# parlance/ctcdecode

Hardware: AMD Instinct MI355X
Metric: utterances/sec at B=256 T=1000 V=29 beam=100 (higher is better)
Workload: dtype f32

## Files before the change

ctcdecode_amd/csrc/beam_core.h:

```cpp
#pragma once
#include <stddef.h>
#include <stdint.h>

#include "exact_math.h"
#include "exact_math_f64.h"
#include "lm_tables.h"
#include "stl_emul.h"
#if defined(CTC_ASSUME_CHECKED)
#include <cstdio>
#include <cstdlib>
#endif

#define CTC_RARE(x) __builtin_expect(!!(x), 0)
#if !defined(CTC_SPEC_UP)
#define CTC_SPEC_UP 1.5f
#endif
#if !defined(CTC_SPEC_DN)
#define CTC_SPEC_DN 0.7f
#endif
#if !defined(CTC_SPEC_OVER_SHIFT)
#define CTC_SPEC_OVER_SHIFT 2
#endif
#define CTC_USUAL(x) __builtin_expect(!!(x), 1)

namespace ctcbeam {

struct alignas(16) Int4v { int x, y, z, w; };

struct PoolNode {
  int32_t parent;
  float lpc;
  uint32_t cht;
  CTC_HD int ch() const { const uint32_t c = cht & 0xFFFFu; return c == 0xFFFFu ? -1 : (int)c; }
  CTC_HD static uint32_t pack(int ch, int tstep) { return ((uint32_t)ch & 0xFFFFu) | ((uint32_t)tstep << 16); }
};

struct EkWide { uint64_t k; uint32_t slot, pad; };
template <bool HUGE> struct EkOps;
template <> struct EkOps<false> {
  using E = uint64_t; using Pos = uint16_t;
  CTC_HD static E make(uint64_t key48v, int slot) { return (key48v << 16) | (uint64_t)slot; }
  CTC_HD static uint64_t key(const E &e) { return e >> 16; }
  CTC_HD static int slot(const E &e) { return (int)(e & 0xFFFFu); }
};
template <> struct EkOps<true> {
  using E = EkWide; using Pos = uint32_t;
  CTC_HD static E make(uint64_t key48v, int slot) { E e; e.k = key48v; e.slot = (uint32_t)slot; e.pad = 0; return e; }
  CTC_HD static uint64_t key(const E &e) { return e.k; }
  CTC_HD static int slot(const E &e) { return (int)e.slot; }
};

enum : uint32_t { T_SELF = 0, T_CHILD = 1, T_REVIVED = 2, T_HOLE = 3 };
enum : int { ST_OK = 0, ST_POOL_OVERFLOW = 1, ST_BAD_CONFIG = 2 };

constexpr int kMaxBeam = 16383;
constexpr int kMaxVocab = 65534;
constexpr int kIntMax = 0x7fffffff;

CTC_HD uint32_t ord_f32(float f) {
  const uint32_t u = ctcmath::f32_to_bits(f + 0.0f);
  return u ^ ((uint32_t)((int32_t)u >> 31) | 0x80000000u);
}
CTC_HD uint32_t ord_f32_raw(float f) {
  const uint32_t u = ctcmath::f32_to_bits(f);
  return u ^ ((uint32_t)((int32_t)u >> 31) | 0x80000000u);
}
CTC_HD float unord_f32(uint32_t k) {
  return ctcmath::bits_to_f32((k & 0x80000000u) ? (k ^ 0x80000000u) : ~k);
}
CTC_HD uint32_t mk_info(int ch, uint32_t type, int entry) {
  return ((uint32_t)(0xFFFF - (ch + 1)) << 16) | (type << 14) | (uint32_t)entry;
}
CTC_HD uint32_t info_type(uint32_t info) { return (info >> 14) & 3u; }
CTC_HD int info_entry(uint32_t info) { return (int)(info & 0x3FFFu); }
CTC_HD int info_ch(uint32_t info) { return 0xFFFF - (int)(info >> 16) - 1; }
CTC_HD uint64_t key48(uint32_t skey, uint32_t info) { return ((uint64_t)skey << 16) | (info >> 16); }
constexpr uint32_t kHoleInfo = T_HOLE << 14;

struct Beam {
  int *node, *par, *ch, *dep, *lcp, *via, *viaanc, *viach;
  int *up;
  float *bprev, *nbprev, *score, *lpc;
  int *lmst, *lmcl;
  int *acc_lo, *acc_hi;
  int *dn, *dmlo, *dmhi, *dfc;
  int *spc_lo, *spc_hi;
  int *spst, *spcl;
};
constexpr int kBeamArrays = 13, kBeamArraysLm = 12;

struct Dims {
  int K;
  int V;
  int Vc_max;
  int use_rank_table;
  int lm;
  CTC_HD int S_max() const { return K * (2 + Vc_max); }
};

enum {
  VAR_STATUS = 0, VAR_CUT, VAR_TAUC,
  VAR_INTO,
  VAR_FB0 = 4, VAR_FB1, VAR_FB2, VAR_FB3,
  VAR_TAU = 8, VAR_G, VAR_E,
  VAR_DANGER,
  VAR_PAR0 = 12,
  P_NPIN = 0, P_LCOUNT, P_NMAXKEY, P_NMINKEY, P_NCAND, P_SIZE = 8,
  VAR_SPEC = VAR_PAR0 + 2 * P_SIZE, SP_THR = 0, SP_WLOG, SP_ANCHOR, SP_PRED, SP_BEST, SP_MARGIN, SP_GAP, SP_ROWMAX,
  VAR_ROWMAX = VAR_SPEC + SP_ROWMAX,
  VAR_QSTAT = VAR_SPEC + 9,
  VAR_LMMISS = VAR_SPEC + 8,
  VAR_LMQ = VAR_SPEC + 10,
  VAR_HOTN = VAR_SPEC + 4,
  VAR_COUNT = VAR_SPEC + 12
};
constexpr int kBins = 1024;
constexpr int kBinsLog = 10;
constexpr int kListCap = 128;
constexpr int kSmallK = 128, kSmallV = 32;
constexpr int kMidK = 112, kMidVc = 40, kMidV = 10240;
constexpr int kHotCap = 256;
#if !defined(CTC_SERIAL_CUT)
#define CTC_SERIAL_CUT 12
#endif
constexpr int kSerialCut = CTC_SERIAL_CUT;
constexpr int kExpress = 32;
enum Event { EV_FRAMES, EV_CANDIDATES, EV_EXACT, EV_INTERNAL, EV_PINNED, EV_LPC_UPDATE, EV_DEAD_PARENT, EV_REVIVE_CAND, EV_REVIVED, EV_WALK,
             EV_WALK_HOPS, EV_FAST_SELECT, EV_SINGLE_KEY, EV_BUCKET_KEYS, EV_SPEC_OK, EV_SPEC_UNDER, EV_SPEC_OVER, EV_SPEC_OTHER, EV_SPEC_HOT,
             EV_SLOW_BELOW, EV_SLOW_CROWDED, EV_SLOW_SINGLE, EV_SLOW_ROUNDS, EV_TIE_FRAMES, EV_TIE_KEYS, EV_TIE_BIG, EV_WIDE_LIST, EV_HOT_LIST, EV_COUNT };

struct Work {
  Beam cur, nxt, beam0;
  size_t beam_blk;
  size_t beam_blk_far;
  size_t blk_via, blk_lm;
  int *e, *anc, *ostart, *cstart, *pinr, *revr;
  int *ancbuf, *acntbuf;
  uint32_t *hit;
  float *b_new, *nb_new, *sc_new, *rev_lpc;
  int *cch;
  float *clp;
  float *clpbuf;
  int16_t *rank_of;
  uint32_t *skey, *sinfo, *pos;
  int *surv;
  uint64_t *ek;
  uint16_t *lr;
  uint32_t *wpre;
  int *bins;
  int *hotge;
  int *lcpst;
  uint32_t *list;
  int *lslot;
  uint32_t *bitmap;
  int *fin, *sstack;
  int stage_skey;
  int *apos;
  int *vars;
};

template <class P>
CTC_HD P *carve_ptr(char *&p, size_t count) {
  P *r = reinterpret_cast<P *>(p);
  p += ((count * sizeof(P) + 15) / 16) * 16;
  return r;
}

template <int BIG, bool FARREP = false>
CTC_HD size_t carve(Work &w, char *base, char *far, const Dims &d, size_t *far_bytes) {
  char *p = base;
  char *q = far;
  constexpr bool deep = BIG >= 2;
  constexpr bool huge = BIG >= 3;
  const size_t K = (size_t)d.K, S = (size_t)d.S_max();
  const size_t Kr = ((K * 4 + 15) / 16) * 16;
  Beam *bs[2] = {&w.cur, &w.nxt};
  constexpr bool lm_far = BIG != 0;
  const size_t n_lm = d.lm ? (size_t)kBeamArraysLm : 0;
  w.beam_blk = (size_t)(kBeamArrays - (deep ? 3 : 0) + (lm_far ? 0 : n_lm)) * Kr;
  w.beam_blk_far = ((deep ? 3 : 0) + (lm_far ? n_lm : 0)) * Kr;
  w.blk_via = deep ? w.beam_blk_far : w.beam_blk;
  w.blk_lm = lm_far ? w.beam_blk_far : w.beam_blk;
  for (int i = 0; i < 2; ++i) {
    Beam &b = *bs[i];
    char *f = q + (size_t)i * w.beam_blk_far;
    b.node = carve_ptr<int>(p, K); b.par = carve_ptr<int>(p, K); b.ch = carve_ptr<int>(p, K);
    b.dep = carve_ptr<int>(p, K); b.lcp = carve_ptr<int>(p, K);
    char *&pv3 = deep ? f : p;
    b.via = carve_ptr<int>(pv3, K); b.viaanc = carve_ptr<int>(pv3, K); b.viach = carve_ptr<int>(pv3, K);
    b.up = carve_ptr<int>(p, K);
    b.bprev = carve_ptr<float>(p, K); b.nbprev = carve_ptr<float>(p, K); b.score = carve_ptr<float>(p, K);
    b.lpc = carve_ptr<float>(p, K);
    const size_t Kl = d.lm ? K : 0;
    char *&pl = lm_far ? f : p;
    b.lmst = carve_ptr<int>(pl, Kl); b.lmcl = carve_ptr<int>(pl, Kl); b.acc_lo = carve_ptr<int>(pl, Kl); b.acc_hi = carve_ptr<int>(pl, Kl);
    b.dn = carve_ptr<int>(pl, Kl); b.dmlo = carve_ptr<int>(pl, Kl); b.dmhi = carve_ptr<int>(pl, Kl); b.dfc = carve_ptr<int>(pl, Kl);
    b.spc_lo = carve_ptr<int>(pl, Kl); b.spc_hi = carve_ptr<int>(pl, Kl); b.spst = carve_ptr<int>(pl, Kl); b.spcl = carve_ptr<int>(pl, Kl);
  }
  q += 2 * w.beam_blk_far;
  w.beam0 = w.cur;
  w.e = carve_ptr<int>(p, K); w.ancbuf = carve_ptr<int>(p, 2 * K); w.acntbuf = carve_ptr<int>(p, 2 * K); w.anc = w.ancbuf;
  w.ostart = carve_ptr<int>(p, K);
  w.cstart = carve_ptr<int>(p, K);
  w.pinr = carve_ptr<int>(deep ? q : p, K);
  w.revr = carve_ptr<int>(deep ? q : p, K); w.hit = carve_ptr<uint32_t>(p, 2 * K);
  w.b_new = carve_ptr<float>(p, K); w.nb_new = carve_ptr<float>(p, K); w.sc_new = carve_ptr<float>(p, K);
  w.rev_lpc = carve_ptr<float>(deep ? q : p, K);
  w.cch = carve_ptr<int>(p, (size_t)d.Vc_max);
  w.clpbuf = carve_ptr<float>(p, 2 * (size_t)d.Vc_max); w.clp = w.clpbuf;
  w.rank_of = carve_ptr<int16_t>(p, d.use_rank_table ? (size_t)d.V : 0);
  w.skey = carve_ptr<uint32_t>(deep ? q : p, S);
  w.surv = carve_ptr<int>(p, 3 * K + 4);
  const size_t lcap = (d.K <= kSmallK && d.Vc_max <= kMidVc) ? (size_t)kHotCap + 64 : (size_t)kListCap + 4;
  w.bins = carve_ptr<int>(p, kBins + kBins / 16 + 4); w.list = carve_ptr<uint32_t>(p, lcap);
  w.lslot = carve_ptr<int>(p, lcap);
  w.hotge = carve_ptr<int>(p, lcap > (size_t)kListCap + 4 ? (size_t)kHotCap : 0);
#if defined(CTC_EXP_LCP_TABLE)
  w.lcpst = carve_ptr<int>(p, (lcap > (size_t)kListCap + 4 && !d.lm) ? (size_t)7 * kSmallK : 0);
#else
  w.lcpst = nullptr;
#endif
  w.bitmap = carve_ptr<uint32_t>(huge ? q : p, 2 * ((S + 63) / 64 + 17));
  w.wpre = huge ? carve_ptr<uint32_t>(q, (S + 63) / 64 + 2) : reinterpret_cast<uint32_t *>(w.bins);
  w.fin = carve_ptr<int>(BIG ? q : p, d.lm ? 2 * K : K);
  w.apos = carve_ptr<int>(BIG ? q : p, K);
  w.sstack = carve_ptr<int>(p, 3 * (2 * 32 + 2));
  w.vars = carve_ptr<int>(p, VAR_COUNT);
  w.sinfo = carve_ptr<uint32_t>(p, BIG ? K : S);
  w.pos = carve_ptr<uint32_t>(BIG ? q : p, K + 2);
  char *&rr = (BIG || FARREP) ? q : p;
  w.ek = carve_ptr<uint64_t>(rr, huge ? 2 * S : S); w.lr = carve_ptr<uint16_t>(rr, (2 * S + 2) * (huge ? 2 : 1));
  w.stage_skey = deep ? 0 : 1;
  if (far_bytes) *far_bytes = (size_t)(q - far);
  return (size_t)(p - base);
}

struct StreamState {
  int *hdr;
  int *arrays;
  int finish;
};
enum { SH_FRAMES = 0, SH_N, SH_POOL, SH_WLOG, SH_MAXKEY, SH_DANGER, SH_MINKEY,
       SH_SP_PRED, SH_SP_GAP, SH_SP_MARGIN,
       SH_WORDS = 12 };
constexpr int kStateArrays = 14;
constexpr int kStateArraysLm = kStateArrays + kBeamArraysLm;
CTC_HD int state_arrays(int lm) { return lm ? kStateArraysLm : kStateArrays; }

struct StepIn {
  int t;
  int Vc;
  int blank_rank;
  int identity;
  float blank_prob;
};


CTC_HD int div_p2(int v, int d) { return v >> __builtin_ctz((unsigned)d); }
CTC_HD int ceil_div_p2(int v, int d) { return div_p2(v + d - 1, d); }

CTC_HD double ctc_log_f64(double v) {
  return ctcmath::log_f64(v, ctcmath::tables64());
}

CTC_HD int ceil_log2_u32(uint32_t v) {
  return v <= 1u ? 0 : 32 - __builtin_clz(v - 1u);
}
CTC_HD int ceil_log2_u64(uint64_t v) {
  return v <= 1 ? 0 : 64 - __builtin_clzll(v - 1);
}

struct OutRefs {
  int32_t *tok, *ts;
  float *score;
  int32_t *len;
  int32_t *n_results;
  int K, T_stride;
  int32_t *c_hdr, *c_ent;
  uint32_t *c_rag;
  unsigned *c_count;
  unsigned c_cap;
  int32_t *m_hdr, *m_ent, *m_done;
  uint32_t *m_rag;
  unsigned m_cap;
};
enum : int { ST_COMPACT_OVERFLOW = 3, ST_INPUT_TIMEOUT = 4,
             ST_NEED_HOST = 5,
             ST_CB_DANGER = 6 };

struct SlotCtx {
  const Beam *pb;
  int n, Vnb, brank;
  uint64_t vmagic;
};

template <class X>
struct FullSyncView {
  X &x;
  CTC_HD int tid() const { return x.tid(); }
  CTC_HD int nt() const { return x.nt(); }
  CTC_HD void sync() { x.sync_full(); }
  CTC_HD int uni(int v) const { return x.uni(v); }
  CTC_HD void block_scan_u32(uint32_t mine, uint32_t *base_out, uint32_t *total_out) { x.block_scan_u32(mine, base_out, total_out); }
  CTC_HD int lanes() const { return x.lanes(); }
  CTC_HD auto ballot(bool p) const { return x.ballot(p); }
  template <class M> CTC_HD int count(M m) const { return x.count(m); }
  template <class M> CTC_HD int count_below(M m) const { return x.count_below(m); }
  CTC_HD uint32_t first_lane(uint32_t v) const { return x.first_lane(v); }
};

#if defined(CTC_ASSUME_CHECKED)
#define CTC_ASSUME(c) do { if (!(c)) { std::fprintf(stderr, "beam_core.h:%d: assumption violated: %s\n", __LINE__, #c); std::abort(); } } while (0)
#elif defined(__clang__)
#define CTC_ASSUME(c) __builtin_assume(c)
#else
#define CTC_ASSUME(c) do { if (!(c)) __builtin_unreachable(); } while (0)
#endif

template <class X, bool IDENT, int SMALLV = 0, bool LM = false, bool LAZY = false, bool FARREP = LAZY, bool HUGE = false, bool WORDLM = false, bool CB = false>
struct Decoder {
  using EO = EkOps<HUGE>;
  using Ek = typename EO::E;
  using LrT = typename EO::Pos;
  static constexpr int kClsK = SMALLV == 2 ? kMidK : kSmallK, kClsVc = SMALLV == 2 ? kMidVc : kSmallV, kClsSlots = kClsK * (2 + kClsVc);
  CTC_HD Ek *ekp() const { return reinterpret_cast<Ek *>(w.ek); }
  CTC_HD LrT *lrp() const { return reinterpret_cast<LrT *>(w.lr); }
  X &x;
  Work &w;
  const Dims d;
  const int blank;
  PoolNode *pool;
  int *pool_up;
  int *pool_thi;
  bool long_t = false;
  const int pool_cap;
  const uint64_t *tbl;
  const ctclm::LmView *lm;

  CTC_HD Decoder(X &x_, Work &w_, const Dims &d_, int blank_, PoolNode *pool_, int *pool_up_, int pool_cap_, const uint64_t *tbl_,
                 const ctclm::LmView *lm_ = nullptr)
      : x(x_), w(w_), d(d_), blank(blank_), pool(pool_), pool_up(pool_up_), pool_thi(pool_up_ + pool_cap_), pool_cap(pool_cap_), tbl(tbl_), lm(lm_) {
    if (LM) {
      const ctclm::DictNode root = lm->dict[0];
      root_lo = (int)root.mask_lo; root_hi = (int)root.mask_hi; root_fc = (int)root.first_child;
      lm_char_v = lm->char_based != 0; lm_wide_v = lm->dict_wide != 0; lm_space = lm->space_id;
      lm_alpha = lm->alpha; lm_beta = lm->beta;
      lm_dict = lm->dict;
    }
  }
  CTC_HD int node_tstep(const PoolNode &pn, int id) const { return (int)(pn.cht >> 16) | (CTC_RARE(long_t) ? pool_thi[id] << 16 : 0); }
  CTC_HD void set_node_time(int id, int ch, int tstep, float lpc) const {
    pool[id].lpc = lpc;
    pool[id].cht = PoolNode::pack(ch, tstep);
    if (CTC_RARE(long_t)) pool_thi[id] = tstep >> 16;
  }

  CTC_HD float lse(float a, float b) const { return ctcmath::lse(a, b, tbl); }

  static constexpr bool kRankEpoch = SMALLV == 2 && !IDENT && X::kRankEpoch;
  CTC_HD static int16_t rank_tag(int t, int r) { return (int16_t)(uint16_t)((((uint32_t)t & 1023u) << 6) | (uint32_t)r); }
  static constexpr bool kTailZero = IDENT && SMALLV && !LAZY && X::kZeroKeyTail;
  CTC_HD void zero_key_tail(int from) {
    if (!kTailZero) return;
    for (int i = from + x.tid(); i < kClsSlots; i += x.nt()) w.skey[i] = 0u;
  }

  static constexpr bool kSpec = SMALLV && (!LM || (X::kSpecLm && !CB)) && !LAZY && X::kSpecSelect;
#if defined(CTC_EXP_HOT_PRELIST)
  static constexpr bool kHotPre = LAZY && !LM && !SMALLV && !HUGE;
#else
  static constexpr bool kHotPre = false;
#endif
  struct HotPre { uint32_t thr; int cap; uint32_t *key; int *slot; };
  uint32_t st_gap = 0;
  uint32_t hot_anchor = 0;
  static constexpr bool kA1Overlap = kSpec && X::kA1Overlap;
  static constexpr bool kLcpTable = kSpec && X::kLcpTable;
  static constexpr bool kParentRec = !SMALLV && !LM && X::kParentRec && !kHotPre;
  static constexpr bool kLmOverlap = LM && WORDLM && SMALLV && !CB && !LAZY && X::kLmOverlap;
  static constexpr uint32_t kLmSpaceDeferred = 0x80000000u;
  CTC_HD void spec_learn(bool selected, uint32_t tau, int hot, int K) const {
    int *sp = w.vars + VAR_SPEC;
    const int pred = sp[SP_PRED];
    const float best = ctcmath::bits_to_f32((uint32_t)sp[SP_BEST]);
    float margin = ctcmath::bits_to_f32((uint32_t)sp[SP_MARGIN]);
    const uint32_t anchor = (uint32_t)sp[SP_ANCHOR];
    int wl = 32;
    float cut = 0.f;
    if (selected) {
      if (pred) {
        if (hot < K) margin = margin < 32.f ? margin * CTC_SPEC_UP : margin;
        else if (hot > K + (K >> CTC_SPEC_OVER_SHIFT) + 3) margin = margin > 0.001f ? margin * CTC_SPEC_DN : margin;
      }
      cut = (best - unord_f32(tau)) + margin;
      const uint32_t kgap = anchor > tau ? anchor - tau : 0u;
      wl = (kgap ? 32 - __builtin_clz(kgap) : 0) + 1;
      wl = wl < kBinsLog ? kBinsLog : (wl > 32 ? 32 : wl);
    }
    sp[SP_MARGIN] = (int)ctcmath::f32_to_bits(margin); sp[SP_GAP] = (int)ctcmath::f32_to_bits(cut);
    sp[SP_PRED] = selected ? 1 : 0; sp[SP_WLOG] = wl;
  }
  CTC_HD void spec_predict(int t) const {
    int *sp = w.vars + VAR_SPEC;
    const int pred = sp[SP_PRED];
    const float rowmax = ctcmath::bits_to_f32((uint32_t)sp[SP_ROWMAX]), cut = ctcmath::bits_to_f32((uint32_t)sp[SP_GAP]);
    const uint32_t mk = (uint32_t)pvars(t - 1)[P_NMAXKEY];
    const float best = unord_f32(mk) + rowmax;
    uint32_t k = ord_f32(best - cut);
    k = k ? k : 1u;
    k = pred ? k : 0xFFFFFFFFu;
    sp[SP_THR] = (int)k; sp[SP_BEST] = (int)ctcmath::f32_to_bits(best); sp[SP_ANCHOR] = (int)mk;
  }

  int st_n = 1, st_pool = 1, st_wlog = 32;
  uint32_t st_maxkey = 0;
  uint32_t st_minkey = 0;
  int root_lo = 0, root_hi = 0, root_fc = 0;
  bool lm_char_v = false, lm_wide_v = false;
  CTC_HD bool lm_char_() const { return !WORDLM && lm_char_v; }
  CTC_HD bool lm_wide_() const { return !WORDLM && lm_wide_v; }
  int lm_space = -1;
  double lm_alpha = 0.0, lm_beta = 0.0;
  const ctclm::DictNode *lm_dict = nullptr;
  static constexpr bool lm_cb = LM && CB;
  CTC_HD int *fin_cur() const { return w.fin + (lm_cb ? st_par * d.K : 0); }
  CTC_HD int *fin_nxt() const { return w.fin + (lm_cb ? (st_par ^ 1) * d.K : 0); }
  CTC_HD double lm_cond_(uint32_t *st, int *cl, uint32_t word, bool *missed = nullptr) const {
    const uint32_t st0 = *st;
    const int cl0 = *cl;
    const double v = ctclm::lm_cond(*lm, st, cl, word);
    if (CTC_RARE(lm_cb)) {
      if (v != v) {
        w.vars[VAR_LMMISS] = 1;
        unsigned i = x.global_add(lm->cb_count, 1u);
        if (lm->cb_ring) i &= lm->cb_cap - 1;
        if (i < lm->cb_cap) lm->cb_miss[i] = ctclm::MissEntry{st0, word, (uint32_t)x.item(), 1u};
        x.atomic_add(&w.vars[VAR_LMQ], 1);
        *st = st0; *cl = cl0;
        if (missed) *missed = true;
        return 0.0;
      }
      if (v == -__builtin_huge_val()) return ctclm::kOovScore;
    }
    return v;
  }
  static constexpr int kLmPending = -1;
  int st_par = 0;

  template <class P>
// ... 535 lines not shown
#else
    (void)hp;
    if (CTC_USUAL(fb[0] >= 0 && fb[3] <= kListCap && (wd.shift != 0 || fb[0] == kBins - 1))) {
      const uint32_t b32 = wd.lo + ((uint32_t)fb[0] << wd.shift);
      const uint32_t bspan = fb[0] == kBins - 1 ? 0xFFFFFFFFu - b32 : (1u << wd.shift) - 1u;
      if (tid == 0) { x.count(EV_FAST_SELECT, 1); x.count(EV_BUCKET_KEYS, fb[3]); if (fb[3] == 1) x.count(EV_SINGLE_KEY, 1); }
      if (kHotPre) {
        const int hot_n = x.uni(w.vars[VAR_HOTN]);
        const bool from_hot = hp.thr != 0xFFFFFFFFu && hp.thr <= b32 && hot_n <= hp.cap;
        if (tid == 0 && from_hot) x.count(EV_HOT_LIST, 1);
        rank_bucket_ext(S, pv, b32, bspan, true, K - fb[1], fb[1], fb[3], w.list, w.lslot, from_hot ? &hp : nullptr, hot_n);
      } else {
        rank_bucket(S, pv, b32, bspan, true, K - fb[1], fb[1], fb[3]);
      }
      return true;
    }
#endif
    uint64_t lo = wd.lo, hi = (uint64_t)1 << 32;
    int shift = wd.shift;
    int need = K, gbase = 0;
    bool first = true;
    for (;;) {
      const int bstar = fb[0], above = fb[1], total = fb[2], inb = fb[3];
      uint64_t blo = 0, bhi = 0;
      bool again = true;
      if (tid == 0) x.count(EV_SLOW_ROUNDS, 1);
      if (bstar < 0) {
        if (tid == 0) x.count(EV_SLOW_BELOW, 1);
        gbase += total; need -= total; hi = lo; lo = 1;
      } else {
        blo = lo + ((uint64_t)bstar << shift);
        bhi = (bstar == kBins - 1) ? hi : blo + ((uint64_t)1 << shift);
        if (bhi > hi) bhi = hi;
        if (shift == 0 && bstar < kBins - 1) {
          if (tid == 0) x.count(EV_SLOW_SINGLE, 1);
          if (tid == 0) { w.vars[VAR_TAU] = (int)(uint32_t)blo; w.vars[VAR_G] = gbase + above; w.vars[VAR_E] = inb; }
          x.sync();
          return false;
        }
        if (inb <= kListCap) again = false;
        else { if (tid == 0) x.count(EV_SLOW_CROWDED, 1); gbase += above; need -= above; lo = blo; hi = bhi; }
      }
      if (!again) {
        rank_bucket<true>(S, pv, (uint32_t)blo, (uint32_t)(bhi - blo - 1), first, need - above, gbase + above, inb);
        return first;
      }
      first = false;
      for (int i = tid; i < kBins; i += nt) w.bins[i] = 0;
      x.sync();
      const uint64_t width = hi - lo;
      shift = width <= (uint64_t)kBins ? 0 : ceil_log2_u64(width) - kBinsLog;
      const uint32_t lo32 = (uint32_t)lo, span = (uint32_t)(hi - lo - 1);
      for (int s0 = tid; s0 < S; s0 += 4 * nt) {
        uint32_t kk[4];
        for (int u = 0; u < 4; ++u) kk[u] = s0 + u * nt < S ? w.skey[s0 + u * nt] : 0u;
        for (int u = 0; u < 4; ++u) {
          const uint32_t k = kk[u], dk = k - lo32;
          if (k >= lo32 && dk <= span) {
            const uint32_t bk = dk >> shift;
            const int bb = bk < (uint32_t)(kBins - 1) ? (int)bk : kBins - 1;
            x.atomic_add(&w.bins[bb], 1);
          }
        }
      }
      x.sync();
      x.find_bucket(w.bins, need, &w.vars[VAR_FB0]);
      x.uni4(&w.vars[VAR_FB0], fb);
    }
  }

  CTC_HD bool resolve_by_character(int S, uint32_t tau, int m, int E, int *pv, const SlotCtx *lz = nullptr) {
    const int tid = x.tid(), nt = x.nt();
    if (E > kListCap) return false;
    if (tid == 0) { pv[P_LCOUNT] = 0; w.vars[VAR_CUT] = 0; }
    x.sync();
    for (int s = tid; s < S; s += nt)
      if (w.skey[s] == tau) w.list[x.atomic_add(&pv[P_LCOUNT], 1)] = ((LAZY ? info_of_slot(*lz, s) : w.sinfo[s]) >> 16) + 1u;
    x.sync();
    for (int q = tid; q < E; q += nt) {
      const uint32_t mine = w.list[q];
      int g = 0, e = 0;
      for (int r = 0; r < E; ++r) {
        const uint32_t o = w.list[r];
        g += o > mine;
        e += o == mine;
      }
      if (g < m && m <= g + e) { w.vars[VAR_TAUC] = (int)(mine - 1u); w.vars[VAR_CUT] = (g + e == m) ? 1 : 2; }
    }
    x.sync();
    return x.uni(w.vars[VAR_CUT]) == 1;
  }

  CTC_HD void build_lcp_table(const Beam &b, int n, int lane) const {
    int *st = w.lcpst;
    const int i0 = lane, i1 = lane + 64;
    int v0 = i0 < n ? b.lcp[i0] : kIntMax, v1 = i1 < n ? b.lcp[i1] : kIntMax;
    st[i0] = v0; st[i1] = v1;
    x.wave_lds_fence();
#if defined(__clang__)
#pragma unroll
#endif
    for (int l = 1; l <= 6; ++l) {
      const int h = 1 << (l - 1);
      const int *p = st + (l - 1) * kSmallK;
      const int a = p[i0 + h];
      const int c = i1 + h < kSmallK ? p[i1 + h] : kIntMax;
      v0 = a < v0 ? a : v0; v1 = c < v1 ? c : v1;
      st[l * kSmallK + i0] = v0; st[l * kSmallK + i1] = v1;
      x.wave_lds_fence();
    }
  }
  CTC_HD int lca_depth_tbl(int ja, int jb) const {
    const int lo = ja < jb ? ja : jb, hi = ja < jb ? jb : ja;
    const int len = hi - lo;
    const int l = 31 - __builtin_clz((unsigned)(len > 0 ? len : 1));
    const int *p = w.lcpst + l * kSmallK;
    const int same = w.cur.dep[ja];
    const int a = p[lo + 1 < kSmallK ? lo + 1 : kSmallK - 1], c = p[hi - (1 << l) + 1];
    const int m = a < c ? a : c;
    return len == 0 ? same : m;
  }
  CTC_HD int lca_depth(int ja, int jb) const {
    const Beam &b = w.cur;
    if (ja == jb) return b.dep[ja];
    const int lo = ja < jb ? ja : jb, hi = ja < jb ? jb : ja;
    int m = kIntMax;
    for (int i = lo + 1; i <= hi; i += 8) {
      const int i1 = i + 1 < hi ? i + 1 : hi, i2 = i + 2 < hi ? i + 2 : hi, i3 = i + 3 < hi ? i + 3 : hi;
      const int i4 = i + 4 < hi ? i + 4 : hi, i5 = i + 5 < hi ? i + 5 : hi, i6 = i + 6 < hi ? i + 6 : hi, i7 = i + 7 < hi ? i + 7 : hi;
      const int l0 = b.lcp[i], l1 = b.lcp[i1], l2 = b.lcp[i2], l3 = b.lcp[i3];
      const int l4 = b.lcp[i4], l5 = b.lcp[i5], l6 = b.lcp[i6], l7 = b.lcp[i7];
      const int m01 = l0 < l1 ? l0 : l1, m23 = l2 < l3 ? l2 : l3, m45 = l4 < l5 ? l4 : l5, m67 = l6 < l7 ? l6 : l7;
      const int ma = m01 < m23 ? m01 : m23, mb = m45 < m67 ? m45 : m67;
      const int mm = ma < mb ? ma : mb;
      m = mm < m ? mm : m;
    }
    return m;
  }

  template <class XX>
  CTC_HD int hoare_round(XX &xx, Ek *v, int first, int last, LrT *Lp, LrT *Rp) {
    if (FARREP) return stlemu::hoare_round_parallel<true>(xx, v, first, last, [](const Ek &e) { return EO::key(e); }, Lp, Rp, &w.vars[VAR_CUT]);
    return stlemu::hoare_round_parallel_chunks(xx, v, first, last, [](const Ek &e) { return EO::key(e); }, Lp, Rp, &w.vars[VAR_CUT]);
  }

  template <class XX>
  CTC_HD bool replay_nth_element(XX &fx, int N, int K) {
    const int tid = x.tid(), nt = x.nt();
    Ek *v = ekp();
    LrT *lr = lrp();
    auto before = [](const Ek &a, const Ek &c) { return EO::key(a) > EO::key(c); };
    int first = 0, last = N, depth = 2 * stlemu::floor_lg(N);
    if (!FARREP) {
      while (last - first > kSerialCut && depth > 0) {
        --depth;
        const int cut = hoare_round(x, v, first, last, lr, lr + N + 1);
        if (cut <= K) first = cut; else last = cut;
      }
      if (tid == 0) stlemu::introselect(v, first, K, last, depth, before);
      x.sync();
      return false;
    }
    Ek *sv = reinterpret_cast<Ek *>(w.nxt.node);
    int stage_cap = (int)((w.beam_blk - 16) / (sizeof(Ek) + 2 * sizeof(LrT)));
    if (w.stage_skey) {
      sv = reinterpret_cast<Ek *>(w.skey);
      const int cap_e = d.S_max() / 2, cap_p = (int)(w.beam_blk / 4) - 2;
      stage_cap = cap_e < cap_p ? cap_e : cap_p;
    }
    while (last - first > kSerialCut && depth > 0 && last - first > stage_cap) {
      --depth;
      const int cut = hoare_round(fx, v, first, last, lr, lr + N + 1);
      if (cut <= K) first = cut; else last = cut;
    }
    if (last - first > kSerialCut && depth > 0) {
      const int m0 = last - first, base = first;
      LrT *sLp = w.stage_skey ? reinterpret_cast<LrT *>(w.nxt.node) : reinterpret_cast<LrT *>(sv + m0), *sRp = sLp + m0 + 1;
      for (int i = tid; i < m0; i += nt) sv[i] = v[base + i];
      x.sync();
      int f2 = 0, l2 = m0;
      const int K2 = K - base;
      while (l2 - f2 > kSerialCut && depth > 0) {
        --depth;
        const int cut = hoare_round(x, sv, f2, l2, sLp, sRp);
        if (cut <= K2) f2 = cut; else l2 = cut;
      }
      if (tid == 0) stlemu::introselect(sv, f2, K2, l2, depth, before);
      x.sync();
      for (int i = tid; i < m0; i += nt) v[base + i] = sv[i];
      fx.sync();
      return w.stage_skey != 0;
    }
    if (tid == 0) stlemu::introselect(v, first, K, last, depth, before);
    fx.sync();
    return false;
  }

  CTC_HD void prime_a1(int t) {
    if (!kA1Overlap) return;
    select_beams();
    phase_a1(w.cur, st_n, w.ancbuf + (t & 1) * d.K, w.acntbuf + (t & 1) * d.K, x.group(), x.ngroups());
    x.sync();
  }
  CTC_HD void phase_a1(const Beam &b, int n, int *anc, int *acnt, int grp, int ngr) {
    const int rows = ceil_div_p2(n, ngr);
    auto entry_of = [=](int r) { return r * ngr + ((grp - r) & (ngr - 1)); };
    for (int k0 = 0; k0 < rows; k0 += x.lanes()) {
      const int k = k0 + x.lane();
      const int j = entry_of(k);
      bool internal = false;
      int dj = 0;
      if (k < rows && j < n) {
        dj = b.dep[j];
        internal = j + 1 < n && b.lcp[j + 1] >= dj;
        if (!internal) w.e[j] = j + 1;
      }
      unsigned long long todo = x.ballot(internal);
      if (internal) x.count(EV_INTERNAL, 1);
      if ((LM || (X::kQuarters && __builtin_popcountll(todo) >= 3)) && x.subtrees_by_quarters(todo, k0, grp, ngr, b.dep, b.lcp, n, w.e, anc, acnt)) todo = 0;
      while (todo) {
        const int kk = __builtin_ctzll(todo);
        todo &= todo - 1;
        const int jj = entry_of(k0 + kk);
        const int q = x.first_below(b.lcp, jj + 2, n, x.pick(dj, kk));
        if (x.lane() == 0) w.e[jj] = q;
        for (int c = jj + 1 + x.lane(); c < q; c += x.lanes()) {
          x.atomic_max(&anc[c], jj);
          x.atomic_add(&acnt[c], 1);
        }
      }
    }
  }

  CTC_HD int step(const StepIn &in, bool last, bool stage = false, float stage_val = 0.f, int next_cnt = 0, float next_val = 0.f) {
    select_beams();
    const Beam b = w.cur;
    const Beam nb = w.nxt;
    const int tid = x.tid_fresh(), nt = x.nt();
    const int n = st_n, pool_count = st_pool;
    const int K = d.K;
    const int Vc = in.Vc, brank = in.blank_rank;
    if (SMALLV) { CTC_ASSUME(n >= 1 && n <= kClsK); CTC_ASSUME(Vc >= 1 && Vc <= kClsVc); CTC_ASSUME(d.K <= kClsK); }
    const int Vnb = Vc - (brank >= 0 ? 1 : 0);
    const int S = n * (2 + Vnb);
    const bool small_vocab = SMALLV || Vnb <= 64;
    int *pv = pvars(in.t);
    int *surv = w.surv, *rk = w.surv + K, *ord = w.surv + 2 * K;
    Window wd{1u, 0};
    if (!kSpec) wd = first_window();
    HotPre hp{0xFFFFFFFFu, 0, nullptr, nullptr};
    if (kHotPre) {
      hp.cap = wide_list_cap();
      hp.key = reinterpret_cast<uint32_t *>(w.nxt.node);
      hp.slot = reinterpret_cast<int *>(hp.key + hp.cap + 4);
      if (x.tid() == 0) w.vars[VAR_HOTN] = 0;
    }
    float min_cutoff = CTC_NEG_MAX;
    bool full_beam = false;
    if (LM) {
      const double bpos = lm_beta > 0.0 ? lm_beta : 0.0;
      min_cutoff = (float)((double)(unord_f32(st_minkey) + in.blank_prob) - bpos);
      full_beam = n == K;
    }
    auto cut = [&](float lp, float prefix_score) { return LM && full_beam && lp + prefix_score < min_cutoff; };
    if (LM && CTC_RARE(x.uni(w.vars[VAR_DANGER]) != 0)) {
      lm_sorted_order(b, n);
    }

    w.anc = w.ancbuf + (in.t & 1) * K;
    int *acnt = w.acntbuf + (in.t & 1) * K;
    const bool lm_job = LM && !lm_char_();
    const int lm_joff = (SMALLV && x.nt_is(1024)) ? kSmallK : nt >= 2 * ((n + 63) & ~63) ? ((n + 63) & ~63) : 0;
    int lm_jk = -1;
    bool lm_defer = false;
    ctclm::DictNode lm_jinfo;
    if (lm_job) {
      const int k = tid - lm_joff;
      if (k >= 0 && k < n) {
        const int fc = b.dfc[k], dnk = b.dn[k];
        if (fc == kLmPending) {
          lm_jk = k; lm_jinfo = lm_dict[dnk];
          if (kLmOverlap) lm_defer = !(k + 1 < n && b.lcp[k + 1] >= b.dep[k]);
        }
      }
    }
    x.tick();
    if (!kA1Overlap) {
      phase_a1(b, n, w.anc, acnt, x.group(), x.ngroups());
      x.tick();
      x.sync();
    }
    if (kSpec && tid == x.spec_thread()) spec_predict(in.t);
    int npin = 0;
    Int4v *prec = reinterpret_cast<Int4v *>(w.nxt.node);
    for (int j = tid; j < n; j += nt) {
      const int dj = b.dep[j], q = w.e[j], P = w.anc[j], a = acnt[j];
      w.ostart[j] = 2 * j + Vnb * (j - a);
      const int cs_j = 2 * q + Vnb * (q - 1 - a);
      w.cstart[j] = cs_j;
      if (kParentRec) prec[j] = Int4v{(int)ctcmath::f32_to_bits(b.score[j]), (int)ctcmath::f32_to_bits(b.bprev[j]), cs_j, b.ch[j]};
      int pr = -1, rr = -1;
      if (P >= 0) {
        if (b.dep[P] == dj - 1) {
          pr = rank_of_char(in, b.ch[j]);
        } else {
          if (CTC_RARE(b.viaanc[j] != b.node[P])) {
            int hops = dj - b.dep[P] - 1, xn = b.node[j];
            x.count(EV_WALK, 1); x.count(EV_WALK_HOPS, hops);
#if !defined(CTC_NO_WALK_FROM_PARENT)
            int h0 = 0;
            if (LM && hops >= 1) { xn = b.par[j]; h0 = 1; }
            for (int h = h0; h < hops; ++h) xn = pool[xn].parent;
// ... 1068 lines not shown
```

ctcdecode_amd/csrc/stl_emul.h:

```cpp
#pragma once
#include <stdint.h>

#if defined(__HIPCC__)
#define STLEMU_HD __host__ __device__ inline
#else
#define STLEMU_HD inline
#endif
#if defined(__HIP_DEVICE_COMPILE__)
#define STLEMU_FN __host__ __device__ __attribute__((noinline))
#else
#define STLEMU_FN STLEMU_HD
#endif

namespace stlemu {

STLEMU_HD int floor_lg(int n) {
  int k = 0;
  while (n > 1) {
    n >>= 1;
    ++k;
  }
  return k;
}

// ... 159 lines not shown
  for (;;) {
    while (last - first > 16) {
      if (depth == 0) {
        heap_select(v, first, last, last, before);
        heap_sort_down(v, first, last, before);
        break;
      }
      --depth;
      int cut = split_with_median_pivot(v, first, last, before);
      stack[sp++] = cut;
      stack[sp++] = last;
      stack[sp++] = depth;
      last = cut;
    }
    if (sp == 0) break;
    depth = stack[--sp];
    last = stack[--sp];
    first = stack[--sp];
  }
  first = lo0;
  last = hi0;
  if (last - first > 16) {
    insertion_sort(v, first, first + 16, before);
    for (int i = first + 16; i != last; ++i) linear_insert_unguarded(v, i, before);
  } else {
    insertion_sort(v, first, last, before);
  }
}

template <class X, class T, class C, class I>
STLEMU_HD void sort_parallel(X &x, T *v, int n, C before, I *cur, I *nxt, I *small, int *cnt, int seeded_tasks = -1,
                             int limit = 0x7fffffff) {
  const int tid = x.tid(), nt = x.nt();
  int ntask = seeded_tasks;
  if (seeded_tasks < 0) {
    if (tid == 0) {
      cnt[0] = 0; cnt[1] = 0; cnt[2] = 0;
      cur[0] = (I)0; cur[1] = (I)n; cur[2] = (I)(2 * floor_lg(n));
    }
    x.sync();
    ntask = 1;
  }
  for (int round = 0; ntask > 0; ++round) {
    int *c_next = cnt + (round & 1);
    for (int k = tid; k < ntask; k += nt) {
      const int first = (int)cur[3 * k], last = (int)cur[3 * k + 1], depth = (int)cur[3 * k + 2];
      if (depth == 0) {
        heap_select(v, first, last, last, before);
        heap_sort_down(v, first, last, before);
        continue;
      }
      const int cut = split_with_median_pivot(v, first, last, before);
      for (int side = 0; side < 2; ++side) {
        const int a = side ? cut : first, e = side ? last : cut;
        if (a >= limit) continue;
        if (e - a > 16) {
          const int i = x.atomic_add(c_next, 1);
          nxt[3 * i] = (I)a; nxt[3 * i + 1] = (I)e; nxt[3 * i + 2] = (I)(depth - 1);
        } else if (e - a > 1) {
          const int i = x.atomic_add(cnt + 2, 1);
          small[2 * i] = (I)a; small[2 * i + 1] = (I)e;
        }
      }
    }
    x.sync();
    ntask = x.uni(*c_next);
    if (tid == 0) cnt[(round + 1) & 1] = 0;
    I *t = cur; cur = nxt; nxt = t;
    x.sync();
  }
  const int nsmall = x.uni(cnt[2]);
  for (int k = tid; k < nsmall; k += nt) insertion_sort(v, (int)small[2 * k], (int)small[2 * k + 1], before);
  x.sync();
}

template <bool MEDIAN_BY_ALL = false, class X, class T, class KeyOf, class P>
STLEMU_HD int hoare_round_parallel(X &x, T *v, int first, int last, KeyOf key_of, P *Lp, P *Rp, int *cutvar) {
  const int tid = x.tid(), nt = x.nt();
  constexpr bool wide = sizeof(P) > 2;
  auto before = [&](const T &a, const T &b) { return key_of(a) > key_of(b); };
  const int lo = first + 1, m = last - lo;
  decltype(key_of(v[first])) kp;
  if (MEDIAN_BY_ALL) {
    const int pa = first + 1, pb = first + (last - first) / 2, pc = last - 1;
    const T va = v[pa], vb = v[pb], vc = v[pc], vf = v[first];
    int pm;
    if (before(va, vb)) pm = before(vb, vc) ? pb : (before(va, vc) ? pc : pa);
    else pm = before(va, vc) ? pa : (before(vb, vc) ? pc : pb);
    const T vm = pm == pa ? va : (pm == pb ? vb : vc);
    x.sync();
    if (tid == 0) { v[first] = vm; v[pm] = vf; }
    x.sync();
    kp = key_of(vm);
  } else {
    if (tid == 0) median_to(v, first, first + 1, first + (last - first) / 2, last - 1, before);
    x.sync();
    kp = key_of(v[first]);
  }
  const int W = x.lanes(), lane = tid % W, grp = tid / W, ng = nt / W;
  const int per = ((m + ng - 1) / ng + W - 1) / W * W;
  const int g0 = grp * per < m ? grp * per : m, g1 = g0 + per < m ? g0 + per : m;
  uint32_t mineL = 0, mineR = 0;
  for (int i = g0; i < g1; i += W) {
    const bool in = i + lane < g1;
    const auto k = in ? key_of(v[lo + i + lane]) : kp;
    mineL += (uint32_t)x.count(x.ballot(in && k <= kp));
    mineR += (uint32_t)x.count(x.ballot(in && k >= kp));
  }
  uint32_t runL, runR;
  int nL, nR;
  if (wide) {
    uint32_t totL, totR;
    x.block_scan_u32(lane == 0 ? mineL : 0u, &runL, &totL);
    x.block_scan_u32(lane == 0 ? mineR : 0u, &runR, &totR);
    nL = (int)totL; nR = (int)totR;
  } else {
    uint32_t run, tot;
    x.block_scan_u32(lane == 0 ? (mineL | (mineR << 16)) : 0u, &run, &tot);
    runL = run & 0xFFFFu; runR = run >> 16;
    nL = (int)(tot & 0xFFFFu); nR = (int)(tot >> 16);
  }
  runL = x.first_lane(runL); runR = x.first_lane(runR);
  for (int i = g0; i < g1; i += W) {
    const bool in = i + lane < g1;
    const auto k = in ? key_of(v[lo + i + lane]) : kp;
    const bool isL = in && k <= kp, isR = in && k >= kp;
    const auto bl = x.ballot(isL), br = x.ballot(isR);
    if (isL) Lp[runL + (uint32_t)x.count_below(bl)] = (P)(lo + i + lane);
    if (isR) Rp[nR - 1 - (int)(runR + (uint32_t)x.count_below(br))] = (P)(lo + i + lane);
    runL += (uint32_t)x.count(bl);
    runR += (uint32_t)x.count(br);
  }
  if (tid == 0) Rp[nR] = (P)first;
  x.sync();
  const int tmax = nL < nR + 1 ? nL : nR + 1;
  auto crossed = [&](int t) { return t >= nL || t > nR || Lp[t] >= Rp[t]; };
  for (int t = tid; t <= tmax; t += nt) {
    if (!crossed(t)) {
      exch(v, (int)Lp[t], (int)Rp[t]);
    } else if (t == 0 || !crossed(t - 1)) {
      int c = t < nL ? (int)Lp[t] : 0x7fffffff;
      if (t > 0 && (int)Rp[t - 1] < c) c = (int)Rp[t - 1];
      *cutvar = c;
    }
  }
  x.sync();
  return x.uni(*cutvar);
}

template <class X, class T, class KeyOf, class P>
STLEMU_HD int hoare_round_parallel_chunks(X &x, T *v, int first, int last, KeyOf key_of, P *Lp, P *Rp, int *cutvar) {
  const int tid = x.tid(), nt = x.nt();
  constexpr bool wide = sizeof(P) > 2;
  auto before = [&](const T &a, const T &b) { return key_of(a) > key_of(b); };
  if (tid == 0) median_to(v, first, first + 1, first + (last - first) / 2, last - 1, before);
  x.sync();
  const int lo = first + 1, m = last - lo;
  const auto kp = key_of(v[first]);
  const int chunk = (m + nt - 1) / nt, i0 = tid * chunk < m ? tid * chunk : m, i1 = i0 + chunk < m ? i0 + chunk : m;
  uint32_t mineL = 0, mineR = 0;
  for (int i = i0; i < i1; ++i) {
    const auto k = key_of(v[lo + i]);
    mineL += k <= kp ? 1u : 0u;
    mineR += k >= kp ? 1u : 0u;
  }
  uint32_t runL, runR;
  int nL, nR;
  if (wide) {
    uint32_t totL, totR;
    x.block_scan_u32(mineL, &runL, &totL);
    x.block_scan_u32(mineR, &runR, &totR);
    nL = (int)totL; nR = (int)totR;
  } else {
    uint32_t run, tot;
    x.block_scan_u32(mineL | (mineR << 16), &run, &tot);
    runL = run & 0xFFFFu; runR = run >> 16;
    nL = (int)(tot & 0xFFFFu); nR = (int)(tot >> 16);
  }
  for (int i = i0; i < i1; ++i) {
    const auto k = key_of(v[lo + i]);
    if (k <= kp) { Lp[runL] = (P)(lo + i); runL += 1u; }
    if (k >= kp) { Rp[nR - 1 - (int)runR] = (P)(lo + i); runR += 1u; }
  }
  if (tid == 0) Rp[nR] = (P)first;
  x.sync();
  const int tmax = nL < nR + 1 ? nL : nR + 1;
  auto crossed = [&](int t) { return t >= nL || t > nR || Lp[t] >= Rp[t]; };
  for (int t = tid; t <= tmax; t += nt) {
    if (!crossed(t)) {
      exch(v, (int)Lp[t], (int)Rp[t]);
    } else if (t == 0 || !crossed(t - 1)) {
      int c = t < nL ? (int)Lp[t] : 0x7fffffff;
      if (t > 0 && (int)Rp[t - 1] < c) c = (int)Rp[t - 1];
      *cutvar = c;
    }
  }
  x.sync();
  return x.uni(*cutvar);
}

template <class X, class T, class KeyOf>
STLEMU_HD void sort_prefix_parallel(X &x, T *v, int n, int limit, int big_cut, KeyOf key_of, uint16_t *Lp, uint16_t *Rp, uint16_t *cur,
                                    uint16_t *nxt, uint16_t *small, int *cnt, int *bstack) {
  const int tid = x.tid();
  auto before = [&](const T &a, const T &b) { return key_of(a) > key_of(b); };
  if (n <= 16) {
    if (tid == 0) sort(v, 0, n, before, bstack);
    x.sync();
    return;
  }
  int sp = 0, ntask = 0, nsmall = 0;
  if (tid == 0) { bstack[0] = 0; bstack[1] = n; bstack[2] = 2 * floor_lg(n); }
  sp = 1;
  x.sync();
  while (sp > 0) {
    --sp;
    const int first = x.uni(bstack[3 * sp]), last = x.uni(bstack[3 * sp + 1]);
    int depth = x.uni(bstack[3 * sp + 2]);
    x.sync();
    if (last - first <= big_cut) {
      if (tid == 0) { cur[3 * ntask] = (uint16_t)first; cur[3 * ntask + 1] = (uint16_t)last; cur[3 * ntask + 2] = (uint16_t)depth; }
      ++ntask;
      continue;
    }
    if (depth == 0) {
      if (tid == 0) { heap_select(v, first, last, last, before); heap_sort_down(v, first, last, before); }
      x.sync();
      continue;
    }
    --depth;
    const int cut = hoare_round_parallel(x, v, first, last, key_of, Lp, Rp, cnt + 3);
    for (int side = 0; side < 2; ++side) {
      const int a = side ? cut : first, e = side ? last : cut;
      if (a >= limit) continue;
      if (e - a > 16) {
        if (tid == 0) { bstack[3 * sp] = a; bstack[3 * sp + 1] = e; bstack[3 * sp + 2] = depth; }
        ++sp;
      } else if (e - a > 1) {
        if (tid == 0) { small[2 * nsmall] = (uint16_t)a; small[2 * nsmall + 1] = (uint16_t)e; }
        ++nsmall;
      }
    }
    x.sync();
  }
  if (tid == 0) { cnt[0] = 0; cnt[1] = 0; cnt[2] = nsmall; }
  x.sync();
  sort_parallel(x, v, n, before, cur, nxt, small, cnt, ntask, limit);
}

template <class T, class C>
STLEMU_HD void partial_sort(T *v, int first, int middle, int last, C before) {
  heap_select(v, first, middle, last, before);
  heap_sort_down(v, first, middle, before);
}

}
```

Measured before the change: 52210.

## Finish nth_element selection with single-wave Hoare rounds instead of serial introselect

The block-wide Hoare partition loop in the non-far replay path now stops at a larger cut (256 elements). A single wavefront finishes the selection using ballot-based partition rounds, with lane 0 running serial introselect only on the last few elements. Previously thread 0 did all of that serially. The block-wide round also computes the median-of-three pivot in every thread, which removes one block barrier per round. This trades block syncs and serial work for wave-local LDS fences, and depends on the pivot swap staying consistent with the equal-key tie handling.

After: 53360, median of 6. +2.2%, better.

```diff
diff --git a/ctcdecode_amd/csrc/beam_core.h b/ctcdecode_amd/csrc/beam_core.h
--- a/ctcdecode_amd/csrc/beam_core.h
+++ b/ctcdecode_amd/csrc/beam_core.h
@@ -124,6 +124,10 @@
 #define CTC_SERIAL_CUT 12
 #endif
 constexpr int kSerialCut = CTC_SERIAL_CUT;
+#if !defined(CTC_WAVE_CUT)
+#define CTC_WAVE_CUT 256
+#endif
+constexpr int kWaveCut = CTC_WAVE_CUT;
 constexpr int kExpress = 32;
 enum Event { EV_FRAMES, EV_CANDIDATES, EV_EXACT, EV_INTERNAL, EV_PINNED, EV_LPC_UPDATE, EV_DEAD_PARENT, EV_REVIVE_CAND, EV_REVIVED, EV_WALK,
              EV_WALK_HOPS, EV_FAST_SELECT, EV_SINGLE_KEY, EV_BUCKET_KEYS, EV_SPEC_OK, EV_SPEC_UNDER, EV_SPEC_OVER, EV_SPEC_OTHER, EV_SPEC_HOT,
@@ -295,6 +299,18 @@
 };
 
 template <class X>
+struct WaveView {
+  X &x;
+  CTC_HD int lane() const { return x.lane(); }
+  CTC_HD int lanes() const { return x.lanes(); }
+  CTC_HD auto ballot(bool p) const { return x.ballot(p); }
+  template <class M> CTC_HD int count(M m) const { return x.count(m); }
+  template <class M> CTC_HD int count_below(M m) const { return x.count_below(m); }
+  template <class M> CTC_HD int ffs(M m) const { return __builtin_ctzll((unsigned long long)m); }
+  CTC_HD void fence() const { x.wave_lds_fence(); }
+};
+
+template <class X>
 struct FullSyncView {
   X &x;
   CTC_HD int tid() const { return x.tid(); }
@@ -1136,12 +1152,15 @@
     auto before = [](const Ek &a, const Ek &c) { return EO::key(a) > EO::key(c); };
     int first = 0, last = N, depth = 2 * stlemu::floor_lg(N);
     if (!FARREP) {
-      while (last - first > kSerialCut && depth > 0) {
+      while (last - first > kWaveCut && depth > 0) {
         --depth;
         const int cut = hoare_round(x, v, first, last, lr, lr + N + 1);
         if (cut <= K) first = cut; else last = cut;
       }
-      if (tid == 0) stlemu::introselect(v, first, K, last, depth, before);
+      if (tid < x.lanes()) {
+        WaveView<X> wv{x};
+        stlemu::introselect_wave(wv, v, first, K, last, depth, [](const Ek &e) { return EO::key(e); }, lr, lr + N + 1);
+      }
       x.sync();
       return false;
     }
diff --git a/ctcdecode_amd/csrc/stl_emul.h b/ctcdecode_amd/csrc/stl_emul.h
--- a/ctcdecode_amd/csrc/stl_emul.h
+++ b/ctcdecode_amd/csrc/stl_emul.h
@@ -335,15 +335,19 @@
 STLEMU_HD int hoare_round_parallel_chunks(X &x, T *v, int first, int last, KeyOf key_of, P *Lp, P *Rp, int *cutvar) {
   const int tid = x.tid(), nt = x.nt();
   constexpr bool wide = sizeof(P) > 2;
-  auto before = [&](const T &a, const T &b) { return key_of(a) > key_of(b); };
-  if (tid == 0) median_to(v, first, first + 1, first + (last - first) / 2, last - 1, before);
-  x.sync();
+  const int pa = first + 1, pb = first + (last - first) / 2, pc = last - 1;
+  const T va = v[pa], vb = v[pb], vc = v[pc], vf = v[first];
+  const auto ka = key_of(va), kb = key_of(vb), kc = key_of(vc);
+  int pm;
+  if (ka > kb) pm = kb > kc ? pb : (ka > kc ? pc : pa);
+  else pm = ka > kc ? pa : (kb > kc ? pc : pb);
+  const T vm = pm == pa ? va : (pm == pb ? vb : vc);
+  const auto kp = key_of(vm), kf = key_of(vf);
   const int lo = first + 1, m = last - lo;
-  const auto kp = key_of(v[first]);
   const int chunk = (m + nt - 1) / nt, i0 = tid * chunk < m ? tid * chunk : m, i1 = i0 + chunk < m ? i0 + chunk : m;
   uint32_t mineL = 0, mineR = 0;
   for (int i = i0; i < i1; ++i) {
-    const auto k = key_of(v[lo + i]);
+    const auto k = lo + i == pm ? kf : key_of(v[lo + i]);
     mineL += k <= kp ? 1u : 0u;
     mineR += k >= kp ? 1u : 0u;
   }
@@ -361,11 +365,15 @@
     nL = (int)(tot & 0xFFFFu); nR = (int)(tot >> 16);
   }
   for (int i = i0; i < i1; ++i) {
-    const auto k = key_of(v[lo + i]);
+    const auto k = lo + i == pm ? kf : key_of(v[lo + i]);
     if (k <= kp) { Lp[runL] = (P)(lo + i); runL += 1u; }
     if (k >= kp) { Rp[nR - 1 - (int)runR] = (P)(lo + i); runR += 1u; }
   }
-  if (tid == 0) Rp[nR] = (P)first;
+  if (tid == 0) {
+    v[first] = vm;
+    v[pm] = vf;
+    Rp[nR] = (P)first;
+  }
   x.sync();
   const int tmax = nL < nR + 1 ? nL : nR + 1;
   auto crossed = [&](int t) { return t >= nL || t > nR || Lp[t] >= Rp[t]; };
@@ -380,6 +388,70 @@
   }
   x.sync();
   return x.uni(*cutvar);
+}
+
+template <class W, class T, class KeyOf, class P>
+STLEMU_HD int hoare_round_wave(W &w, T *v, int first, int last, KeyOf key_of, P *Lp, P *Rq) {
+  const int lane = w.lane(), L = w.lanes();
+  const int pa = first + 1, pb = first + (last - first) / 2, pc = last - 1;
+  const auto ka = key_of(v[pa]), kb = key_of(v[pb]), kc = key_of(v[pc]);
+  int pm;
+  if (ka > kb) pm = kb > kc ? pb : (ka > kc ? pc : pa);
+  else pm = ka > kc ? pa : (kb > kc ? pc : pb);
+  const T vm = v[pm], vf = v[first];
+  w.fence();
+  if (lane == 0) { v[first] = vm; v[pm] = vf; Rq[0] = (P)first; }
+  w.fence();
+  const auto kp = key_of(vm);
+  const int lo = first + 1, m = last - lo;
+  int nL = 0, nR = 0;
+  for (int i = 0; i < m; i += L) {
+    const int at = lo + i + lane;
+    const bool in = i + lane < m;
+    const auto k = in ? key_of(v[at]) : kp;
+    const bool isL = in && k <= kp, isR = in && k >= kp;
+    const auto bl = w.ballot(isL), br = w.ballot(isR);
+    if (isL) Lp[nL + w.count_below(bl)] = (P)at;
+    if (isR) Rq[1 + nR + w.count_below(br)] = (P)at;
+    nL += w.count(bl);
+    nR += w.count(br);
+  }
+  w.fence();
+  for (int t0 = 0;; t0 += L) {
+    const int t = t0 + lane;
+    bool crossed = true;
+    int a = 0, b = 0;
+    if (t < nL && t <= nR) {
+      a = (int)Lp[t];
+      b = (int)Rq[nR - t];
+      crossed = a >= b;
+    }
+    const auto bc = w.ballot(crossed);
+    if (!crossed) {
+      const T ea = v[a], eb = v[b];
+      v[a] = eb;
+      v[b] = ea;
+    }
+    if (bc) {
+      const int ts = t0 + w.ffs(bc);
+      int c = ts < nL ? (int)Lp[ts] : 0x7fffffff;
+      if (ts > 0 && (int)Rq[nR - ts + 1] < c) c = (int)Rq[nR - ts + 1];
+      w.fence();
+      return c;
+    }
+  }
+}
+
+template <class W, class T, class KeyOf, class P>
+STLEMU_HD void introselect_wave(W &w, T *v, int first, int nth, int last, int depth, KeyOf key_of, P *Lp, P *Rq) {
+  while (last - first > 3 && depth > 0) {
+    --depth;
+    const int cut = hoare_round_wave(w, v, first, last, key_of, Lp, Rq);
+    if (cut <= nth) first = cut;
+    else last = cut;
+  }
+  if (w.lane() == 0) introselect(v, first, nth, last, depth, [&](const T &a, const T &b) { return key_of(a) > key_of(b); });
+  w.fence();
 }
 
 template <class X, class T, class KeyOf>
```
